# Jonetz/TreeDetection

Hardware: AMD Instinct MI355X
Metric: tiles/sec (1000x1000 RGB+nDSM) predict_tiles model stage (higher is better)
Workload: dtype f32

## Files before the change

### include/treedet.h

```cpp
#ifndef TREEDET_H
#define TREEDET_H

#include <stddef.h>
#include <stdint.h>

#ifdef __cplusplus
extern "C" {
#endif

typedef int td_status;
typedef struct td_engine td_engine;

enum {
    TD_OK = 0,
    TD_ERR_INVALID = -1,
    TD_ERR_HIP = -2,
    TD_ERR_WEIGHTS = -3,
    TD_ERR_CAPACITY = -4,
    TD_ERR_STATE = -5,
    TD_ERR_UNSUPPORTED = -6
};

enum { TD_PRECISION_FP32 = 0, TD_PRECISION_FP16 = 1 };
enum { TD_INPUT_F32_CHW = 0,
// ... 40 lines not shown
                            const int32_t* hw_out, int B, int Hp, int Wp, void* stream, td_detections* out);
#define TD_PHASE_STEM 6
td_status td_engine_forward_phase(td_engine* e, int phase, const void* images, int input_format, const int32_t* hw_valid,
                                  const int32_t* hw_out, int B, int Hp, int Wp, void* stream, td_detections* out);
td_status td_engine_tensor(td_engine* e, const char* name, void** dev_ptr, int64_t dims[4], int* elem_size);
td_status td_engine_read_tensor(td_engine* e, const char* name, void* dst_dev, int64_t bytes, void* stream);
#define TD_PROF_CATEGORIES 9
td_status td_engine_profile_enable(td_engine* e, int enable);
td_status td_engine_profile_read(td_engine* e, double* ms, int64_t* launches, double* flops, double* bytes, int reset);
#define TD_PROF_CLASSES 7
#define TD_CLS_WINO_GEMM 0
#define TD_CLS_WINO_XFORM 1
#define TD_CLS_CONV1X1 2
#define TD_CLS_CONV3X3 3
#define TD_CLS_FC 4
#define TD_CLS_MASK_HEAD 5
#define TD_CLS_TAIL 6
#define TD_PEAK_F32_MFMA_TFLOPS 157.3
#define TD_PEAK_F16_MFMA_TFLOPS 2500.0
#define TD_HBM_ACHIEVABLE_TBS 6.3
td_status td_engine_profile_classes(td_engine* e, double* ms, int64_t* launches, double* exec_flops, double* bytes, double* tmin_ms, int reset);
const char* td_last_error(void);
void td_engine_destroy(td_engine* e);

td_status td_resize_tile_u8(const uint8_t* src, int h, int w, int c, uint8_t* dst, int out_h, int out_w,
                            int dst_pitch_px, void* tmp_dev , void* stream);
td_status td_resize_batch_u8(const uint8_t* const* src_tiles, int n, int h, int w, int c, uint8_t* dst, int out_h,
                             int out_w, int dst_pitch_px, int64_t dst_image_stride_bytes, void* tmp_dev, void* stream);
td_status td_resize_bilinear_f64(const double* src, int c, int h, int w, float* dst, int out_h, int out_w, int dst_pitch_px,
                                 int64_t dst_plane_stride, void* stream);
td_status td_windows_u16_to_input(const uint16_t* raster, int height, int width, int c, const int32_t* windows, int n, int32_t* band1_max,
                                  float* dst, int out_h, int out_w, int dst_pitch_px, int64_t dst_plane_stride, int64_t dst_image_stride,
                                  void* stream);
void td_resize_shape(int h, int w, int short_edge, int max_size, int* out_h, int* out_w);

td_status td_bottleneck_tail_nhwc(const void* x, const void* w2, const float* scale2, const float* bias2, const void* w3,
                                  const float* scale3, const float* bias3, const void* shortcut, void* y, int B, int H, int W,
                                  int mid, int cout, int precision, void* stream);
td_status td_conv2d_nhwc(const void* x, const void* w, const float* scale, const float* bias,
                         const void* residual, int res_shift, void* y, int B, int H, int W, int Cin,
                         int Cout, int KH, int KW, int stride, int pad, int relu, int precision,
                         void* stream);
td_status td_conv2d_head_nhwc(const void* x, const void* w, const float* bias, const void* head_w, const float* head_b,
                              float* head_y, int B, int H, int W, int Cin, int KH, int KW, int pad, int head_n, int precision,
                              void* stream);
td_status td_conv2d_winograd_nhwc(const float* x, const float* w, const float* scale, const float* bias, float* y, int B,
                                  int H, int W, int Cin, int Cout, int relu, void* stream);
td_status td_conv2d_winograd_head_nhwc(const float* x, const float* w, const float* bias, const float* head_w, const float* head_b,
                                       float* head_y, int B, int H, int W, int Cin, int head_n, void* stream);
td_status td_nms(const float* boxes, const float* scores, int n, float iou_thresh, int32_t* keep_idx,
                 int32_t* keep_count, void* stream);
td_status td_roi_align(const void* feat, int H, int W, int C, const float* rois, int R, float spatial_scale,
                       int pooled, void* out, int precision, void* stream);
td_status td_paste_masks(const float* mask_probs, const float* boxes, int n, int out_h, int out_w,
                         float thresh, int32_t* mask_region, int64_t* mask_offset, uint32_t* mask_bits,
                         int64_t mask_words_cap, void* stream);

td_status td_paste_masks_batch(const float* mask_probs, const float* boxes, const int32_t* counts, const int32_t* out_hw,
                               int batch, int dets_per_image, float thresh, int32_t* mask_region, int64_t* mask_offset,
                               uint32_t* mask_bits, int64_t mask_words_per_image, void* stream);

#define TD_CONTOUR_MAX 256
td_status td_trace_contours_dev(const int32_t* mask_region, const int64_t* mask_offset, const uint32_t* mask_bits,
                                int64_t mask_words_per_image, const int32_t* counts, int batch, int dets_per_image,
                                int16_t* points, int points_cap, int32_t* image_points, int32_t* det_info,
                                int32_t* contour_info, void* stream);

int td_find_contours(const uint8_t* img, int h, int w, int32_t* points, int max_points, int32_t* starts,
                     int max_contours);
int td_tile_polygons_json(const int32_t* mask_region, const int64_t* mask_offset, const uint32_t* mask_bits,
                          int64_t mask_words, const float* scores, const int32_t* classes, int n,
                          const double* transform, const char* image_id, char* buf, int64_t cap, int64_t* needed);

int td_tile_prediction_file(int device, const int32_t* mask_region, const int64_t* mask_offset, const uint32_t* mask_bits_dev,
                            uint32_t* rows_host, int64_t mask_words, const float* scores, const int32_t* classes, int n,
                            const double* transform, const char* image_id, const char* path, int64_t* bytes_written);

int td_batch_prediction_files(int device, int n_tiles, int dets_per_image, const int32_t* mask_region, const int64_t* mask_offset,
                              const uint32_t* mask_bits_dev, uint32_t* rows_host, int64_t bits_stride_words, const float* scores,
                              const int32_t* classes, const int32_t* counts, const double* transforms, const char* image_id,
                              const char* const* paths, int threads, int32_t* status, int64_t* bytes_written);

int64_t td_tiff_lzw_decode(const uint8_t* src, int64_t n, uint8_t* dst, int64_t cap);
int64_t td_tiff_packbits_decode(const uint8_t* src, int64_t n, uint8_t* dst, int64_t cap);
int64_t td_tiff_lzw_encode(const uint8_t* src, int64_t n, uint8_t* dst, int64_t cap);
td_status td_tiff_lzw_decode_dev(const uint8_t* comp, const int64_t* block_off, const int64_t* block_nbytes, int nblocks,
                                 uint8_t* blocks_out, int64_t block_cap, int64_t* decoded, int32_t* status, void* stream);
td_status td_tiff_inflate_dev(const uint8_t* comp, const int64_t* block_off, const int64_t* block_nbytes, int nblocks,
                              uint8_t* blocks_out, int64_t block_cap, int64_t* decoded, int32_t* status, void* stream);
td_status td_tiff_inflate_verified_dev(const uint8_t* comp, const int64_t* block_off, const int64_t* block_nbytes, int nblocks,
                                       uint8_t* blocks_out, int64_t block_cap, int64_t* decoded, int32_t* status, int64_t* end_off,
                                       void* stream);
td_status td_tiff_adler32_blocks_dev(const uint8_t* blocks, int64_t block_cap, const int64_t* decoded, const uint8_t* comp,
                                     const int64_t* block_off, const int64_t* block_nbytes, const int64_t* end_off, int nblocks,
                                     int32_t* status, void* stream);
td_status td_adler32_dev(const uint8_t* data_dev, int64_t n, uint32_t* out_dev, void* stream);
int64_t td_tiff_inflate(const uint8_t* src, int64_t n, uint8_t* dst, int64_t cap);
int64_t td_tiff_inflate_verified(const uint8_t* src, int64_t n, uint8_t* dst, int64_t cap);
td_status td_tiff_blocks_to_image_dev(const uint8_t* blocks, int64_t block_cap, int block_w, int block_h, int blocks_across,
                                      int blocks_down, int spp, int predictor, uint8_t* image, int width, int height, void* stream);
td_status td_tiff_blocks_to_image_u16_dev(const uint8_t* blocks, int64_t block_cap, int block_w, int block_h, int blocks_across,
                                          int blocks_down, int spp, int predictor, uint16_t* image, int width, int height, void* stream);
td_status td_tiff_blocks_to_image_f32_dev(const uint8_t* blocks, int64_t block_cap, int block_w, int block_h, int blocks_across,
                                          int blocks_down, int spp, int predictor, float* image, int width, int height, void* stream);
#define TD_JPEG_TABSET_BYTES 11904
td_status td_tiff_jpeg_plan(const uint8_t* tables, int64_t tables_len, const uint8_t* data, const int64_t* block_off,
// ... 55 lines not shown
```

### treedetection_amd/_lib.py

```python
from __future__ import annotations

import ctypes as C
import os
import threading
from typing import Optional

_HERE = os.path.dirname(os.path.abspath(__file__))
LIB_PATH = os.path.join(_HERE, "libtreedet_hip.so")

_lib: Optional[C.CDLL] = None
ERR_INVALID = -1
ERR_CAPACITY = -4
ERR_STATE = -5
ERR_UNSUPPORTED = -6
JPEG_TABSET_BYTES = 11904
SAMPLE_U8, SAMPLE_F32 = 0, 1
RESAMPLE_MODES = {"f32": 0, "u8": 1, "ndvi": 2}


class TdError(RuntimeError):
    """A libtreedet_hip call returned a negative status (message from td_last_error)."""


class ModelDesc(C.Structure):
    _fields_ = [("num_classes", C.c_int32), ("precision", C.c_int32), ("pre_nms_topk", C.c_int32),
                ("post_nms_topk", C.c_int32), ("detections_per_image", C.c_int32),
                ("rpn_nms_thresh", C.c_float), ("score_thresh", C.c_float), ("nms_thresh", C.c_float),
                ("mask_thresh", C.c_float)]


class TensorDesc(C.Structure):
    _fields_ = [("name", C.c_char_p), ("data", C.c_void_p), ("ndim", C.c_int32), ("shape", C.c_int64 * 4)]


class Detections(C.Structure):
    _fields_ = [("boxes", C.c_void_p), ("scores", C.c_void_p), ("classes", C.c_void_p), ("count", C.c_void_p),
                ("mask_probs", C.c_void_p), ("mask_region", C.c_void_p), ("mask_offset", C.c_void_p),
                ("mask_bits", C.c_void_p), ("mask_words_per_image", C.c_int64)]


SIGNATURES = {
    "td_model_desc_default": (None, [C.POINTER(ModelDesc)]),
    "td_engine_create": (C.c_int, [C.POINTER(ModelDesc), C.c_int, C.POINTER(C.c_void_p)]),
    "td_engine_load_weights": (C.c_int, [C.c_void_p, C.POINTER(TensorDesc), C.c_size_t]),
    "td_engine_reserve": (C.c_int, [C.c_void_p, C.c_int, C.c_int, C.c_int]),
    "td_engine_forward": (C.c_int, [C.c_void_p, C.c_void_p, C.c_int, C.POINTER(C.c_int32), C.POINTER(C.c_int32),
                                    C.c_int, C.c_int, C.c_int, C.c_void_p, C.POINTER(Detections)]),
    "td_engine_forward_phase": (C.c_int, [C.c_void_p, C.c_int, C.c_void_p, C.c_int, C.POINTER(C.c_int32), C.POINTER(C.c_int32),
                                          C.c_int, C.c_int, C.c_int, C.c_void_p, C.POINTER(Detections)]),
    "td_engine_tensor": (C.c_int, [C.c_void_p, C.c_char_p, C.POINTER(C.c_void_p), C.POINTER(C.c_int64),
                                   C.POINTER(C.c_int)]),
    "td_engine_read_tensor": (C.c_int, [C.c_void_p, C.c_char_p, C.c_void_p, C.c_int64, C.c_void_p]),
    "td_engine_profile_enable": (C.c_int, [C.c_void_p, C.c_int]),
    "td_engine_profile_read": (C.c_int, [C.c_void_p, C.POINTER(C.c_double), C.POINTER(C.c_int64), C.POINTER(C.c_double),
                                         C.POINTER(C.c_double), C.c_int]),
    "td_engine_profile_classes": (C.c_int, [C.c_void_p, C.POINTER(C.c_double), C.POINTER(C.c_int64), C.POINTER(C.c_double),
                                            C.POINTER(C.c_double), C.POINTER(C.c_double), C.c_int]),
    "td_last_error": (C.c_char_p, []),
    "td_engine_destroy": (None, [C.c_void_p]),
    "td_resize_tile_u8": (C.c_int, [C.c_void_p, C.c_int, C.c_int, C.c_int, C.c_void_p, C.c_int, C.c_int, C.c_int,
                                    C.c_void_p, C.c_void_p]),
    "td_resize_batch_u8": (C.c_int, [C.POINTER(C.c_void_p), C.c_int, C.c_int, C.c_int, C.c_int, C.c_void_p, C.c_int, C.c_int,
                                     C.c_int, C.c_int64, C.c_void_p, C.c_void_p]),
    "td_bottleneck_tail_nhwc": (C.c_int, [C.c_void_p] * 9 + [C.c_int] * 6 + [C.c_void_p]),
    "td_resize_bilinear_f64": (C.c_int, [C.c_void_p, C.c_int, C.c_int, C.c_int, C.c_void_p, C.c_int, C.c_int, C.c_int, C.c_int64, C.c_void_p]),
    "td_windows_u16_to_input": (C.c_int, [C.c_void_p, C.c_int, C.c_int, C.c_int, C.c_void_p, C.c_int, C.c_void_p, C.c_void_p, C.c_int, C.c_int,
                                          C.c_int, C.c_int64, C.c_int64, C.c_void_p]),
    "td_resize_shape": (None, [C.c_int, C.c_int, C.c_int, C.c_int, C.POINTER(C.c_int), C.POINTER(C.c_int)]),
    "td_conv2d_nhwc": (C.c_int, [C.c_void_p, C.c_void_p, C.c_void_p, C.c_void_p, C.c_void_p, C.c_int, C.c_void_p]
                       + [C.c_int] * 11 + [C.c_void_p]),
    "td_conv2d_head_nhwc": (C.c_int, [C.c_void_p] * 6 + [C.c_int] * 9 + [C.c_void_p]),
    "td_conv2d_winograd_head_nhwc": (C.c_int, [C.c_void_p] * 6 + [C.c_int] * 5 + [C.c_void_p]),
    "td_conv2d_winograd_nhwc": (C.c_int, [C.c_void_p] * 5 + [C.c_int] * 6 + [C.c_void_p]),
    "td_nms": (C.c_int, [C.c_void_p, C.c_void_p, C.c_int, C.c_float, C.c_void_p, C.c_void_p, C.c_void_p]),
    "td_roi_align": (C.c_int, [C.c_void_p, C.c_int, C.c_int, C.c_int, C.c_void_p, C.c_int, C.c_float, C.c_int,
                               C.c_void_p, C.c_int, C.c_void_p]),
    "td_paste_masks": (C.c_int, [C.c_void_p, C.c_void_p, C.c_int, C.c_int, C.c_int, C.c_float, C.c_void_p,
                                 C.c_void_p, C.c_void_p, C.c_int64, C.c_void_p]),
    "td_paste_masks_batch": (C.c_int, [C.c_void_p, C.c_void_p, C.c_void_p, C.POINTER(C.c_int32), C.c_int, C.c_int, C.c_float,
                                       C.c_void_p, C.c_void_p, C.c_void_p, C.c_int64, C.c_void_p]),
    "td_crown_stats": (C.c_int, [C.c_void_p, C.c_int, C.c_int, C.POINTER(C.c_double), C.POINTER(C.c_int32), C.c_void_p, C.c_int,
                                 C.c_int, C.c_float, C.c_void_p, C.c_void_p]),
    "td_resample_gdal_dev": (C.c_int, [C.c_void_p, C.c_int, C.c_int, C.c_int, C.c_int, C.POINTER(C.c_int32), C.c_int]
                             + [C.c_void_p] * 4 + [C.c_int, C.c_int64] + [C.c_void_p] * 4 + [C.c_int, C.c_int64]
                             + [C.c_void_p, C.c_void_p, C.c_int, C.c_void_p]),
    "td_crown_pairs_count": (C.c_int, [C.c_void_p, C.c_void_p, C.c_int, C.c_float, C.c_uint16, C.c_void_p, C.c_float, C.c_void_p, C.c_void_p,
                                       C.c_void_p]),
    "td_crown_pairs_fill": (C.c_int, [C.c_void_p, C.c_void_p, C.c_int, C.c_float, C.c_uint16, C.c_void_p, C.c_void_p, C.c_void_p, C.c_void_p]),
    "td_crown_pairs_greedy": (C.c_int, [C.c_void_p, C.c_void_p, C.c_void_p, C.c_void_p, C.c_int, C.c_void_p]),
    "td_trace_contours_dev": (C.c_int, [C.c_void_p, C.c_void_p, C.c_void_p, C.c_int64, C.c_void_p, C.c_int, C.c_int, C.c_void_p,
                                        C.c_int, C.c_void_p, C.c_void_p, C.c_void_p, C.c_void_p]),
    "td_find_contours": (C.c_int, [C.c_void_p, C.c_int, C.c_int, C.c_void_p, C.c_int, C.c_void_p, C.c_int]),
    "td_batch_prediction_files": (C.c_int, [C.c_int, C.c_int, C.c_int, C.c_void_p, C.c_void_p, C.c_void_p, C.c_void_p, C.c_int64, C.c_void_p,
                                          C.c_void_p, C.c_void_p, C.c_void_p, C.c_char_p, C.POINTER(C.c_char_p), C.c_int, C.c_void_p, C.c_void_p]),
    "td_tiff_lzw_decode": (C.c_int64, [C.c_void_p, C.c_int64, C.c_void_p, C.c_int64]),
    "td_tiff_packbits_decode": (C.c_int64, [C.c_void_p, C.c_int64, C.c_void_p, C.c_int64]),
    "td_tiff_lzw_encode": (C.c_int64, [C.c_void_p, C.c_int64, C.c_void_p, C.c_int64]),
    "td_tiff_inflate": (C.c_int64, [C.c_void_p, C.c_int64, C.c_void_p, C.c_int64]),
    "td_tiff_inflate_dev": (C.c_int, [C.c_void_p, C.c_void_p, C.c_void_p, C.c_int, C.c_void_p, C.c_int64, C.c_void_p, C.c_void_p, C.c_void_p]),
    "td_tiff_inflate_verified": (C.c_int64, [C.c_void_p, C.c_int64, C.c_void_p, C.c_int64]),
    "td_tiff_inflate_verified_dev": (C.c_int, [C.c_void_p, C.c_void_p, C.c_void_p, C.c_int, C.c_void_p, C.c_int64, C.c_void_p, C.c_void_p, C.c_void_p,
                                               C.c_void_p]),
    "td_tiff_adler32_blocks_dev": (C.c_int, [C.c_void_p, C.c_int64, C.c_void_p, C.c_void_p, C.c_void_p, C.c_void_p, C.c_void_p, C.c_int, C.c_void_p,
                                             C.c_void_p]),
    "td_adler32_dev": (C.c_int, [C.c_void_p, C.c_int64, C.c_void_p, C.c_void_p]),
    "td_tiff_lzw_decode_dev": (C.c_int, [C.c_void_p, C.c_void_p, C.c_void_p, C.c_int, C.c_void_p, C.c_int64, C.c_void_p, C.c_void_p, C.c_void_p]),
    "td_tiff_blocks_to_image_dev": (C.c_int, [C.c_void_p, C.c_int64, C.c_int, C.c_int, C.c_int, C.c_int, C.c_int, C.c_int, C.c_void_p, C.c_int, C.c_int, C.c_void_p]),
    "td_tiff_blocks_to_image_u16_dev": (C.c_int, [C.c_void_p, C.c_int64, C.c_int, C.c_int, C.c_int, C.c_int, C.c_int, C.c_int, C.c_void_p, C.c_int,
                                                  C.c_int, C.c_void_p]),
    "td_tiff_blocks_to_image_f32_dev": (C.c_int, [C.c_void_p, C.c_int64, C.c_int, C.c_int, C.c_int, C.c_int, C.c_int, C.c_int, C.c_void_p, C.c_int,
                                                  C.c_int, C.c_void_p]),
    "td_tiff_jpeg_plan": (C.c_int, [C.c_void_p, C.c_int64, C.c_void_p, C.c_void_p, C.c_void_p, C.c_int, C.c_int, C.c_int, C.c_int, C.c_void_p,
                                    C.c_void_p, C.c_void_p, C.c_int64, C.c_void_p, C.c_int64, C.c_void_p]),
    "td_tiff_jpeg_decode_dev": (C.c_int, [C.c_void_p, C.c_void_p, C.c_int, C.c_void_p, C.c_int, C.c_void_p, C.c_void_p, C.c_void_p, C.c_int64,
                                          C.c_void_p, C.c_void_p] + [C.c_int] * 6 + [C.c_void_p]),
    "td_jpeg_decode": (C.c_int64, [C.c_void_p, C.c_int64, C.c_void_p, C.c_int64, C.c_void_p]),
    "td_read_windows": (C.c_int64, [C.c_int, C.c_int, C.c_void_p, C.c_int64, C.c_void_p, C.c_void_p, C.c_void_p, C.c_void_p, C.c_int]),
    "td_tiff_unpredict": (C.c_int, [C.c_void_p, C.c_int64, C.c_int64, C.c_int, C.c_int]),
    "td_tiff_unpredict_float": (C.c_int, [C.c_void_p, C.c_int64, C.c_int64, C.c_int, C.c_int]),
    "td_region_relate": (C.c_int, [C.c_void_p, C.c_void_p, C.c_void_p, C.c_int, C.c_void_p, C.c_void_p, C.c_int, C.c_void_p]),
    "td_simplify_ring": (C.c_int, [C.c_void_p, C.c_int, C.c_double, C.c_void_p, C.c_int]),
    "td_ring_is_valid": (C.c_int, [C.c_void_p, C.c_int]),
    "td_stitch_tile_json": (C.c_int, [C.c_char_p, C.c_int64, C.POINTER(C.c_double), C.c_double, C.c_int32, C.c_void_p,
                                      C.c_int64, C.c_void_p, C.c_void_p, C.c_int, C.POINTER(C.c_int64), C.POINTER(C.c_int)]),
    "td_stitch_tile_files": (C.c_int, [C.c_char_p, C.c_void_p, C.c_int, C.c_void_p, C.c_double, C.c_void_p, C.c_int, C.c_void_p, C.c_int64,
                                       C.c_void_p, C.c_void_p, C.c_int, C.c_void_p, C.POINTER(C.c_int64), C.POINTER(C.c_int)]),
    "td_tile_polygons_json_dev": (C.c_int, [C.c_void_p, C.c_int64, C.c_void_p, C.c_void_p, C.c_void_p, C.c_void_p, C.c_void_p, C.c_int64,
                                            C.c_void_p, C.c_void_p, C.c_int, C.POINTER(C.c_double), C.c_char_p, C.c_void_p, C.c_int64,
                                            C.POINTER(C.c_int64)]),
# ... 71 lines not shown
```

### treedetection_amd/csrc/api.cpp

```cpp
#include "common.h"
#include "detect.h"
#include <cstdarg>
#include <cstdio>
#include <cmath>
#include <cstdlib>
#include <vector>


namespace {
td_status scratch(void** p, size_t bytes) {
    TD_HIP_CHECK(hipMalloc(p, bytes ? bytes : 16));
    return TD_OK;
}
}

extern "C" {

void td_model_desc_default(td_model_desc* d) {
    d->num_classes = 1;
    d->precision = TD_PRECISION_FP32;
    d->pre_nms_topk = 1000;
    d->post_nms_topk = 1000;
    d->detections_per_image = 100;
    d->rpn_nms_thresh = 0.7f;
// ... 179 lines not shown
    const double scale = (double)short_edge / (double)(h < w ? h : w);
    double newh, neww;
    if (h < w) { newh = short_edge; neww = scale * w; }
    else { newh = scale * h; neww = short_edge; }
    const double mx = newh > neww ? newh : neww;
    if (mx > max_size) {
        const double s2 = (double)max_size / mx;
        newh *= s2;
        neww *= s2;
    }
    *out_h = (int)(newh + 0.5);
    *out_w = (int)(neww + 0.5);
}

td_status td_nms(const float* boxes, const float* scores, int n, float iou_thresh, int32_t* keep_idx,
                 int32_t* keep_count, void* stream) {
    TD_REQUIRE(boxes && scores && keep_idx && keep_count, "td_nms: null pointer");
    TD_REQUIRE(n >= 0 && n <= 32768, "td_nms: n=%d must be in [0, 32768]", n);
    hipStream_t s = static_cast<hipStream_t>(stream);
    if (n == 0) {
        TD_HIP_CHECK(hipMemsetAsync(keep_count, 0, sizeof(int32_t), s));
        return TD_OK;
    }
    void *sb = nullptr, *ss = nullptr, *si = nullptr, *sc = nullptr, *mk = nullptr, *kp = nullptr;
    td_status st;
    if ((st = scratch(&sb, sizeof(float) * 4 * n)) < 0) return st;
    if ((st = scratch(&ss, sizeof(float) * n)) < 0) return st;
    if ((st = scratch(&si, sizeof(int) * n)) < 0) return st;
    if ((st = scratch(&sc, sizeof(int))) < 0) return st;
    if ((st = scratch(&mk, sizeof(unsigned long long) * n * td_cdiv(n, 64))) < 0) return st;
    if ((st = scratch(&kp, sizeof(int) * n)) < 0) return st;
    if (n > 1024) {
        st = nms_big_launch(boxes, scores, n, iou_thresh, (float*)sb, (float*)ss, (int*)si, (int*)sc, (unsigned long long*)mk, (int*)kp, keep_count, s);
    } else {
        st = sort_boxes_launch(boxes, scores, nullptr, nullptr, 1, n, (float*)sb, (float*)ss, (int*)si, (int*)sc, s);
        if (st >= 0) st = nms_launch((float*)sb, (int*)sc, nullptr, 1, n, iou_thresh, (unsigned long long*)mk, (int*)kp, keep_count, n, s);
    }
    if (st >= 0) st = gather_keep_launch((int*)si, (int*)kp, keep_count, n, keep_idx, s);
    hipError_t herr = hipStreamSynchronize(s);
    (void)hipFree(sb); (void)hipFree(ss); (void)hipFree(si); (void)hipFree(sc); (void)hipFree(mk); (void)hipFree(kp);
    if (st < 0) return st;
    TD_HIP_CHECK(herr);
    return TD_OK;
}

td_status td_roi_align(const void* feat, int H, int W, int C, const float* rois, int R, float spatial_scale,
                       int pooled, void* out, int precision, void* stream) {
    TD_REQUIRE(feat && rois && out, "td_roi_align: null pointer");
    TD_REQUIRE(H >= 1 && W >= 1 && pooled >= 1 && R >= 0, "td_roi_align: bad geometry");
    if (R == 0) return TD_OK;
    return roi_align_single_launch(feat, H, W, C, rois, R, spatial_scale, pooled, out, precision, static_cast<hipStream_t>(stream));
}

td_status td_paste_masks(const float* mask_probs, const float* boxes, int n, int out_h, int out_w, float thresh,
                         int32_t* mask_region, int64_t* mask_offset, uint32_t* mask_bits, int64_t mask_words_cap,
                         void* stream) {
    TD_REQUIRE(mask_probs && boxes && mask_region && mask_offset && mask_bits, "td_paste_masks: null pointer");
    TD_REQUIRE(n >= 0 && n <= 1024 && out_h >= 1 && out_w >= 1, "td_paste_masks: bad shape");
    if (n == 0) return TD_OK;
    hipStream_t s = static_cast<hipStream_t>(stream);
    void* cnt = nullptr;
    td_status st = scratch(&cnt, sizeof(int));
    if (st < 0) return st;
    TD_HIP_CHECK(hipMemcpy(cnt, &n, sizeof(int), hipMemcpyHostToDevice));
    ImgSizes outsz{};
    outsz.h[0] = out_h;
    outsz.w[0] = out_w;
    st = paste_masks_launch(mask_probs, boxes, (int*)cnt, outsz, 1, n, thresh, mask_region,
                            reinterpret_cast<long long*>(mask_offset), mask_bits, mask_words_cap, s);
    hipError_t herr = hipStreamSynchronize(s);
    (void)hipFree(cnt);
    if (st < 0) return st;
    TD_HIP_CHECK(herr);
    return TD_OK;
}

td_status td_paste_masks_batch(const float* mask_probs, const float* boxes, const int32_t* counts, const int32_t* out_hw,
                               int batch, int dets_per_image, float thresh, int32_t* mask_region, int64_t* mask_offset,
                               uint32_t* mask_bits, int64_t mask_words_per_image, void* stream) {
    TD_REQUIRE(mask_probs && boxes && counts && out_hw && mask_region && mask_offset && mask_bits,
               "td_paste_masks_batch: null pointer");
    TD_REQUIRE(batch >= 1 && batch <= TD_MAX_BATCH && dets_per_image >= 1 && dets_per_image <= 1024,
               "td_paste_masks_batch: batch %d (max %d) / detections per image %d (max 1024)", batch, TD_MAX_BATCH, dets_per_image);
    ImgSizes outsz{};
    for (int i = 0; i < batch; ++i) {
        TD_REQUIRE(out_hw[2 * i] >= 1 && out_hw[2 * i + 1] >= 1, "td_paste_masks_batch: bad output size of image %d", i);
        outsz.h[i] = out_hw[2 * i];
        outsz.w[i] = out_hw[2 * i + 1];
        const int64_t need = (int64_t)dets_per_image * ((outsz.w[i] + 2 + 31) / 32) * outsz.h[i];
        TD_REQUIRE(mask_words_per_image >= need, "td_paste_masks_batch: image %d needs %lld mask words, capacity %lld", i,
                   (long long)need, (long long)mask_words_per_image);
    }
    return paste_masks_launch(mask_probs, boxes, counts, outsz, batch, dets_per_image, thresh, mask_region,
                              reinterpret_cast<long long*>(mask_offset), mask_bits, mask_words_per_image,
                              static_cast<hipStream_t>(stream));
}

}
```

### treedetection_amd/csrc/roi.hip

```cpp
#include "common.h"
#include "detect.h"
#include <cstdlib>
#include <type_traits>

namespace {

typedef _Float16 h4 __attribute__((ext_vector_type(4)));
__device__ __forceinline__ float4 load4(const float* p) { return *reinterpret_cast<const float4*>(p); }
__device__ __forceinline__ float4 load4(const _Float16* p) {
    const h4 v = *reinterpret_cast<const h4*>(p);
    return make_float4((float)v[0], (float)v[1], (float)v[2], (float)v[3]);
}
__device__ __forceinline__ void store4(float* p, const float4& v) { *reinterpret_cast<float4*>(p) = v; }
__device__ __forceinline__ void store4(_Float16* p, const float4& v) {
    h4 h;
    h[0] = (_Float16)v.x; h[1] = (_Float16)v.y; h[2] = (_Float16)v.z; h[3] = (_Float16)v.w;
    *reinterpret_cast<h4*>(p) = h;
}

__device__ __forceinline__ int fpn_level(float x1, float y1, float x2, float y2) {
    const float area = __fmul_rn(__fsub_rn(x2, x1), __fsub_rn(y2, y1));
    const float s = sqrtf(area);
    float lv = floorf(__fadd_rn(4.f, log2f(__fadd_rn(__fdiv_rn(s, 224.f), 1e-8f))));
    lv = fminf(fmaxf(lv, 2.f), 5.f);
// ... 13 lines not shown
    int gh, gw, ghw;
    float sh, sw, bh, bw;
    float count;
    size_t feat_off;
    int lvl;
};

__device__ __forceinline__ bool roi_setup(const FeatLevels& fl, const float* __restrict__ rois, const int* __restrict__ counts,
                                          int items, int roi_stride, int pooled, int compact, int* __restrict__ total_rows,
                                          int single_level, int item, int r, RoiGeo& g) {
    const int cnt = counts ? counts[item] : roi_stride;
    int prefix = 0;
    if (compact) {
        for (int i = 0; i < item; ++i) prefix += counts[i];
        if (blockIdx.x == 0 && blockIdx.y == 0 && threadIdx.x == 0 && total_rows) {
            int t = 0;
            for (int i = 0; i < items; ++i) t += counts[i];
            *total_rows = t;
        }
    }
    if (r >= cnt) return false;
    g.row = compact ? (size_t)(prefix + r) : (size_t)item * roi_stride + r;
    const float4 bx = *reinterpret_cast<const float4*>(rois + ((size_t)item * roi_stride + r) * 4);
    g.lvl = single_level ? 0 : fpn_level(bx.x, bx.y, bx.z, bx.w);
    g.H = fl.h[g.lvl];
    g.W = fl.w[g.lvl];
    const float sc = fl.scale[g.lvl];
    g.feat_off = single_level ? 0 : (size_t)item * g.H * g.W * fl.C;
    g.sw = __fsub_rn(__fmul_rn(bx.x, sc), 0.5f);
    g.sh = __fsub_rn(__fmul_rn(bx.y, sc), 0.5f);
    const float ew = __fsub_rn(__fmul_rn(bx.z, sc), 0.5f), eh = __fsub_rn(__fmul_rn(bx.w, sc), 0.5f);
    const float rw = __fsub_rn(ew, g.sw), rh = __fsub_rn(eh, g.sh);
    g.bh = __fdiv_rn(rh, (float)pooled);
    g.bw = __fdiv_rn(rw, (float)pooled);
    int gh = (int)ceilf(__fdiv_rn(rh, (float)pooled)), gw = (int)ceilf(__fdiv_rn(rw, (float)pooled));
    g.gh = gh > 0 ? gh : 0;
    g.gw = gw > 0 ? gw : 0;
    g.ghw = g.gh * g.gw;
    g.count = (float)(g.ghw > 1 ? g.ghw : 1);
    return true;
}

__device__ __forceinline__ bool roi_sample(float start, float bin, int p, int i, int g, int size, int& lo, int& hi, float& l, float& h) {
    const float c = __fadd_rn(__fadd_rn(start, __fmul_rn((float)p, bin)), __fdiv_rn(__fmul_rn(__fadd_rn((float)i, 0.5f), bin), (float)g));
    if (c < -1.f || c > (float)size) return false;
    float cc = c <= 0.f ? 0.f : c;
    lo = (int)cc;
    if (lo >= size - 1) { hi = lo = size - 1; cc = (float)lo; } else hi = lo + 1;
    l = __fsub_rn(cc, (float)lo);
    h = __fsub_rn(1.f, l);
    return true;
}

template <typename T, int D>
__global__ __launch_bounds__(256) void roi_align_kernel(FeatLevels fl, const float* __restrict__ rois,
                                                        const int* __restrict__ counts, int items, int roi_stride,
                                                        int pooled, int compact, T* __restrict__ out,
                                                        int* __restrict__ total_rows, int single_level, int parts) {
    const int item = blockIdx.y, r = blockIdx.x / parts, part = blockIdx.x - r * parts;
    RoiGeo geo;
    if (!roi_setup(fl, rois, counts, items, roi_stride, pooled, compact, total_rows, single_level, item, r, geo)) return;
    const size_t row = geo.row;
    const int H = geo.H, W = geo.W, C = fl.C, gh = geo.gh, gw = geo.gw, ghw = geo.ghw;
    const float sh = geo.sh, sw = geo.sw, bh = geo.bh, bw = geo.bw, count = geo.count;
    const T* __restrict__ feat = static_cast<const T*>(fl.feat[geo.lvl]) + geo.feat_off;

    constexpr int TAB = 14 * 24;
    __shared__ int t_lo[2][TAB], t_hi[2][TAB];
    __shared__ float t_l[2][TAB], t_h[2][TAB];
    const bool tab = pooled * gh <= TAB && pooled * gw <= TAB;
    if (tab) {
        for (int t = threadIdx.x; t < pooled * gh + pooled * gw; t += blockDim.x) {
            const int ax = t < pooled * gh ? 0 : 1;
            const int u = ax ? t - pooled * gh : t;
            const int g = ax ? gw : gh;
            const int p = u / g, i = u - p * g;
            int lo = 0, hi = 0;
            float l = 0.f, h = 0.f;
            const bool ok = ax ? roi_sample(sw, bw, p, i, g, W, lo, hi, l, h) : roi_sample(sh, bh, p, i, g, H, lo, hi, l, h);
            t_lo[ax][u] = ok ? lo : -1;
            t_hi[ax][u] = hi;
            t_l[ax][u] = l;
            t_h[ax][u] = h;
        }
        __syncthreads();
    }

    const int lane = threadIdx.x & 63, wave = __builtin_amdgcn_readfirstlane(threadIdx.x >> 6);
    const int nbins = pooled * pooled;
    const int g0 = part * 4 + wave, gstride = 4 * parts;
#define TD_RA(f) acc.f = __fadd_rn(acc.f, __fadd_rn(__fadd_rn(__fadd_rn(__fmul_rn(w1, v1.f), __fmul_rn(w2, v2.f)), __fmul_rn(w3, v3.f)), __fmul_rn(w4, v4.f)))
    if (tab && ghw > 0) {
        typedef typename Raw4<T>::type R4;
        const int nb_w = g0 < nbins ? (nbins - 1 - g0) / gstride + 1 : 0;
        const int total = nb_w * ghw;
        for (int cb = 0; cb < C; cb += 256) {
            const int c0 = cb + lane * 4;
            const bool act = c0 < C;
            int i_bin = g0, i_iy = 0, i_ix = 0, i_ph = g0 / pooled, i_pw = g0 - (g0 / pooled) * pooled;
            int c_bin = g0, c_n = 0;
            R4 v[D][4];
            float wgt[D][4];
            int ok[D];
            float4 acc = make_float4(0.f, 0.f, 0.f, 0.f);
            const int c0l = act ? c0 : 0;
            const int nb_all = nbins;
            auto issue = [&](int d) {
                const int ph = i_bin < nb_all ? i_ph : 0, pw = i_bin < nb_all ? i_pw : 0;
                const int yi = ph * gh + i_iy, xi = pw * gw + i_ix;
                const int yl = __builtin_amdgcn_readfirstlane(t_lo[0][yi]), xl = __builtin_amdgcn_readfirstlane(t_lo[1][xi]);
                const int yh = __builtin_amdgcn_readfirstlane(t_hi[0][yi]), xh = __builtin_amdgcn_readfirstlane(t_hi[1][xi]);
                ok[d] = yl >= 0 && xl >= 0;
                const float ly = t_l[0][yi], hy = t_h[0][yi], lx = t_l[1][xi], hx = t_h[1][xi];
                wgt[d][0] = __fmul_rn(hy, hx);
                wgt[d][1] = __fmul_rn(hy, lx);
                wgt[d][2] = __fmul_rn(ly, hx);
                wgt[d][3] = __fmul_rn(ly, lx);
                const int syl = ok[d] ? yl : 0, syh = ok[d] ? yh : 0, sxl = ok[d] ? xl : 0, sxh = ok[d] ? xh : 0;
                v[d][0] = *reinterpret_cast<const R4*>(feat + ((size_t)syl * W + sxl) * C + c0l);
                v[d][1] = *reinterpret_cast<const R4*>(feat + ((size_t)syl * W + sxh) * C + c0l);
                v[d][2] = *reinterpret_cast<const R4*>(feat + ((size_t)syh * W + sxl) * C + c0l);
                v[d][3] = *reinterpret_cast<const R4*>(feat + ((size_t)syh * W + sxh) * C + c0l);
                if (++i_ix == gw) {
                    i_ix = 0;
                    if (++i_iy == gh) {
                        i_iy = 0;
                        i_bin += gstride;
                        i_ph = i_bin / pooled;
                        i_pw = i_bin - i_ph * pooled;
                    }
                }
            };
            auto consume = [&](int d) {
                if (ok[d]) {
                    const float w1 = wgt[d][0], w2 = wgt[d][1], w3 = wgt[d][2], w4 = wgt[d][3];
                    const float4 v1 = widen4(v[d][0]), v2 = widen4(v[d][1]), v3 = widen4(v[d][2]), v4 = widen4(v[d][3]);
                    TD_RA(x); TD_RA(y); TD_RA(z); TD_RA(w);
                }
                if (++c_n == ghw) {
                    if (act) {
                        acc.x = __fdiv_rn(acc.x, count);
                        acc.y = __fdiv_rn(acc.y, count);
                        acc.z = __fdiv_rn(acc.z, count);
// ... 346 lines not shown
    const int x0 = rg[0], y0 = rg[1], x1 = rg[2], y1 = rg[3];
    const int wpr = (x1 - x0 + 31) >> 5, rows = y1 - y0;
    if (wpr <= 0 || rows <= 0) return;
    const float4 bx = *reinterpret_cast<const float4*>(boxes + ((size_t)b * D + d) * 4);
    const float bw = __fsub_rn(bx.z, bx.x), bh = __fsub_rn(bx.w, bx.y);
    uint32_t* out = bits + (size_t)b * words_per_image + offset[(size_t)b * D + d];
    for (int wi = threadIdx.x; wi < wpr * rows; wi += blockDim.x) {
        const int ry = wi / wpr, wx = wi - ry * wpr;
        const float py = __fadd_rn((float)(y0 + ry), 0.5f);
        const float gy = __fsub_rn(__fmul_rn(__fdiv_rn(__fsub_rn(py, bx.y), bh), 2.f), 1.f);
        const float iy = __fdiv_rn(__fsub_rn(__fmul_rn(__fadd_rn(gy, 1.f), (float)MS), 1.f), 2.f);
        const float iy0f = floorf(iy);
        const float wn = __fsub_rn(__fadd_rn(iy0f, 1.f), iy), ws = __fsub_rn(iy, iy0f);
        const int iy0 = (int)iy0f, iy1 = iy0 + 1;
        const bool yok0 = iy0 >= 0 && iy0 < MS, yok1 = iy1 >= 0 && iy1 < MS;
        uint32_t word = 0u;
        for (int bit = 0; bit < 32; ++bit) {
            const int x = x0 + wx * 32 + bit;
            if (x >= x1) break;
            const float px = __fadd_rn((float)x, 0.5f);
            const float gx = __fsub_rn(__fmul_rn(__fdiv_rn(__fsub_rn(px, bx.x), bw), 2.f), 1.f);
            const float ix = __fdiv_rn(__fsub_rn(__fmul_rn(__fadd_rn(gx, 1.f), (float)MS), 1.f), 2.f);
            const float ix0f = floorf(ix);
            const float ww = __fsub_rn(__fadd_rn(ix0f, 1.f), ix), we = __fsub_rn(ix, ix0f);
            float v = 0.f;
            if (isfinite(ix) && isfinite(iy)) {
                const int ix0 = (int)ix0f, ix1 = ix0 + 1;
                const bool xok0 = ix0 >= 0 && ix0 < MS, xok1 = ix1 >= 0 && ix1 < MS;
                const float nw = (yok0 && xok0) ? m[iy0 * MS + ix0] : 0.f;
                const float ne = (yok0 && xok1) ? m[iy0 * MS + ix1] : 0.f;
                const float sw = (yok1 && xok0) ? m[iy1 * MS + ix0] : 0.f;
                const float se = (yok1 && xok1) ? m[iy1 * MS + ix1] : 0.f;
                v = __fmul_rn(nw, __fmul_rn(wn, ww));
                v = __fadd_rn(v, __fmul_rn(ne, __fmul_rn(wn, we)));
                v = __fadd_rn(v, __fmul_rn(sw, __fmul_rn(ws, ww)));
                v = __fadd_rn(v, __fmul_rn(se, __fmul_rn(ws, we)));
            }
            if (v >= thresh) word |= 1u << bit;
        }
        out[(size_t)ry * wpr + wx] = word;
    }
}

}

static bool roi_h8_ok(const FeatLevels& fl) {
    static const char* env = getenv("TD_ROI_H8");
    if (env && atoi(env) == 0) return false;
    for (int l = 0; l < ROI_LEVELS; ++l)
        if ((size_t)fl.h[l] * (size_t)fl.w[l] * (size_t)fl.C >= ((size_t)1 << 32)) return false;
    return fl.C <= 256 && fl.C % 8 == 0;
}

template <typename T>
static void roi_align_dispatch(dim3 grid, hipStream_t stream, int depth, const FeatLevels& fl, const float* rois, const int* counts,
                               int items, int roi_stride, int pooled, int compact, T* out, int* total_rows, int single_level, int parts) {
    if constexpr (std::is_same<T, _Float16>::value) {
        if (roi_h8_ok(fl)) {
#define TD_ROI_LAUNCH8(DD) hipLaunchKernelGGL((roi_align_h8_kernel<DD>), grid, dim3(256), 0, stream, fl, rois, counts, items, \
                                              roi_stride, pooled, compact, out, total_rows, single_level, parts)
            switch (depth) {
                case 1: TD_ROI_LAUNCH8(1); break;
                case 3: TD_ROI_LAUNCH8(3); break;
                case 4: TD_ROI_LAUNCH8(4); break;
                default: TD_ROI_LAUNCH8(2); break;
            }
#undef TD_ROI_LAUNCH8
            return;
        }
    }
#define TD_ROI_LAUNCH(DD) hipLaunchKernelGGL((roi_align_kernel<T, DD>), grid, dim3(256), 0, stream, fl, rois, counts, items, \
                                             roi_stride, pooled, compact, out, total_rows, single_level, parts)
    switch (depth) {
        case 1: TD_ROI_LAUNCH(1); break;
        case 2: TD_ROI_LAUNCH(2); break;
        case 3: TD_ROI_LAUNCH(3); break;
        case 6: TD_ROI_LAUNCH(6); break;
        case 8: TD_ROI_LAUNCH(8); break;
        default: TD_ROI_LAUNCH(4); break;
    }
#undef TD_ROI_LAUNCH
}

static int roi_depth(int precision) {
    static const char* env = getenv("TD_ROI_DEPTH");
    if (env) return atoi(env);
    return precision == TD_PRECISION_FP16 ? 2 : 4;
}

static int roi_parts(int pooled) {
    static const char* env = getenv("TD_ROI_PARTS");
    if (env) return atoi(env) > 0 ? atoi(env) : 1;
    return pooled * pooled >= 128 ? 4 : 1;
}

td_status roi_align_launch(const FeatLevels& fl, const float* rois, const int* counts, int items, int roi_stride,
                           int pooled, int compact, void* out, int* total_rows, int precision, hipStream_t stream) {
    TD_REQUIRE(fl.C % 4 == 0, "roi_align: C must be a multiple of 4");
    const int parts = roi_parts(pooled);
    const dim3 grid(roi_stride * parts, items);
    if (precision == TD_PRECISION_FP16)
        roi_align_dispatch<_Float16>(grid, stream, roi_depth(precision), fl, rois, counts, items, roi_stride, pooled, compact,
                                     static_cast<_Float16*>(out), total_rows, 0, parts);
    else
        roi_align_dispatch<float>(grid, stream, roi_depth(precision), fl, rois, counts, items, roi_stride, pooled, compact,
                                  static_cast<float*>(out), total_rows, 0, parts);
    TD_KERNEL_CHECK();
    return TD_OK;
}

td_status roi_align_single_launch(const void* feat, int H, int W, int C, const float* rois, int R, float scale,
                                  int pooled, void* out, int precision, hipStream_t stream) {
    TD_REQUIRE(C % 4 == 0 && R >= 1, "roi_align: bad shape");
    FeatLevels fl{};
    fl.feat[0] = feat; fl.h[0] = H; fl.w[0] = W; fl.scale[0] = scale; fl.C = C;
    const int parts = roi_parts(pooled);
    const dim3 grid(R * parts, 1);
    if (precision == TD_PRECISION_FP16)
        roi_align_dispatch<_Float16>(grid, stream, roi_depth(precision), fl, rois, nullptr, 1, R, pooled, 0,
                                     static_cast<_Float16*>(out), nullptr, 1, parts);
    else
        roi_align_dispatch<float>(grid, stream, roi_depth(precision), fl, rois, nullptr, 1, R, pooled, 0,
                                  static_cast<float*>(out), nullptr, 1, parts);
    TD_KERNEL_CHECK();
    return TD_OK;
}

td_status det_decode_launch(const float* cls_reg, int cr_stride, const float* props, const int* prop_count,
                            const ImgSizes& valid, int B, int prop_stride, float score_thresh, float* boxes,
                            float* scores, int* flags, hipStream_t stream) {
    hipLaunchKernelGGL(det_decode_kernel, dim3(td_cdiv(B * prop_stride, 256)), dim3(256), 0, stream, cls_reg, cr_stride,
                       props, prop_count, valid, B, prop_stride, score_thresh, boxes, scores, flags);
    TD_KERNEL_CHECK();
    return TD_OK;
}

td_status det_finalize_launch(const float* sboxes, const float* sscores, const int* keep_pos, const int* keep_count,
                              const ImgSizes& valid, const ImgSizes& outsz, int B, int stride_items, int max_det,
                              float* det_boxes_net, float* out_boxes, float* out_scores, int* out_classes,
                              int* out_count, hipStream_t stream) {
    hipLaunchKernelGGL(det_finalize_kernel, dim3(B), dim3(64), 0, stream, sboxes, sscores, keep_pos, keep_count, valid,
                       outsz, stride_items, max_det, det_boxes_net, out_boxes, out_scores, out_classes, out_count);
    TD_KERNEL_CHECK();
    return TD_OK;
}

td_status mask_predict_launch(const void* x, const float* w, float bias, int C, int rows_max, const int* rows_dyn,
                              int rows_mul, float* logits_out, float* probs_out, int precision, hipStream_t stream) {
    TD_REQUIRE(C % 4 == 0, "mask_predict: C must be a multiple of 4");
    if (rows_max <= 0) return TD_OK;
    if (precision == TD_PRECISION_FP16)
        hipLaunchKernelGGL((mask_predict_kernel<_Float16>), dim3(td_cdiv(rows_max, 4)), dim3(256), 0, stream,
                           static_cast<const _Float16*>(x), w, bias, C, rows_max, rows_dyn, rows_mul, logits_out, probs_out);
    else
        hipLaunchKernelGGL((mask_predict_kernel<float>), dim3(td_cdiv(rows_max, 4)), dim3(256), 0, stream,
                           static_cast<const float*>(x), w, bias, C, rows_max, rows_dyn, rows_mul, logits_out, probs_out);
    TD_KERNEL_CHECK();
    return TD_OK;
}

td_status mask_scatter_launch(const float* compact, const int* counts, int B, int D, float* out, hipStream_t stream) {
    hipLaunchKernelGGL(mask_scatter_kernel, dim3(D, B), dim3(256), 0, stream, compact, counts, B, D, out);
    TD_KERNEL_CHECK();
    return TD_OK;
}

td_status paste_masks_launch(const float* probs, const float* boxes, const int* counts, const ImgSizes& outsz, int B,
                             int D, float thresh, int* region, long long* offset, uint32_t* bits,
                             long long words_per_image, hipStream_t stream) {
    hipLaunchKernelGGL(paste_plan_kernel, dim3(B), dim3(64), 0, stream, boxes, counts, outsz, D, region, offset,
                       words_per_image);
    TD_KERNEL_CHECK();
    hipLaunchKernelGGL(paste_fill_kernel, dim3(D, B), dim3(256), 0, stream, probs, boxes, counts, D, thresh, region,
                       offset, bits, words_per_image);
    TD_KERNEL_CHECK();
    return TD_OK;
// ... 2 lines not shown
```

Measured before the change: 678.8.

## Add streaming ROI-align path reusing column loads with LDS bin accumulators

Adds a streaming path to the FP32 ROI-align kernel for the case where the x sample table is monotone and densely covers a contiguous column range. Each feature column pair is loaded once per row and scattered into per-bin accumulators held in LDS, in runs of seven bins, instead of re-fetching four corners for every sample. The path is on by default and launches seven waves per block with dynamic LDS, replacing 256-thread blocks. It also exposes a multi-level ROI-align entry point in the C API and ctypes bindings. The trade-offs are more complex control flow, higher LDS use per block, and possibly different occupancy.

```diff
diff --git a/include/treedet.h b/include/treedet.h
--- a/include/treedet.h
+++ b/include/treedet.h
@@ -116,6 +116,9 @@
                  int32_t* keep_count, void* stream);
 td_status td_roi_align(const void* feat, int H, int W, int C, const float* rois, int R, float spatial_scale,
                        int pooled, void* out, int precision, void* stream);
+td_status td_roi_align_levels(const void* const feats[4], const int32_t h[4], const int32_t w[4], const float scale[4], int C,
+                              const float* rois, const int32_t* counts, int items, int roi_stride, int pooled, int compact,
+                              void* out, int32_t* total_rows, int precision, void* stream);
 td_status td_paste_masks(const float* mask_probs, const float* boxes, int n, int out_h, int out_w,
                          float thresh, int32_t* mask_region, int64_t* mask_offset, uint32_t* mask_bits,
                          int64_t mask_words_cap, void* stream);
diff --git a/treedetection_amd/_lib.py b/treedetection_amd/_lib.py
--- a/treedetection_amd/_lib.py
+++ b/treedetection_amd/_lib.py
@@ -75,6 +75,9 @@
     "td_nms": (C.c_int, [C.c_void_p, C.c_void_p, C.c_int, C.c_float, C.c_void_p, C.c_void_p, C.c_void_p]),
     "td_roi_align": (C.c_int, [C.c_void_p, C.c_int, C.c_int, C.c_int, C.c_void_p, C.c_int, C.c_float, C.c_int,
                                C.c_void_p, C.c_int, C.c_void_p]),
+    "td_roi_align_levels": (C.c_int, [C.POINTER(C.c_void_p), C.POINTER(C.c_int32), C.POINTER(C.c_int32), C.POINTER(C.c_float), C.c_int,
+                                      C.c_void_p, C.c_void_p, C.c_int, C.c_int, C.c_int, C.c_int, C.c_void_p, C.c_void_p, C.c_int,
+                                      C.c_void_p]),
     "td_paste_masks": (C.c_int, [C.c_void_p, C.c_void_p, C.c_int, C.c_int, C.c_int, C.c_float, C.c_void_p,
                                  C.c_void_p, C.c_void_p, C.c_int64, C.c_void_p]),
     "td_paste_masks_batch": (C.c_int, [C.c_void_p, C.c_void_p, C.c_void_p, C.POINTER(C.c_int32), C.c_int, C.c_int, C.c_float,
diff --git a/treedetection_amd/csrc/api.cpp b/treedetection_amd/csrc/api.cpp
--- a/treedetection_amd/csrc/api.cpp
+++ b/treedetection_amd/csrc/api.cpp
@@ -255,6 +255,22 @@
     return roi_align_single_launch(feat, H, W, C, rois, R, spatial_scale, pooled, out, precision, static_cast<hipStream_t>(stream));
 }
 
+td_status td_roi_align_levels(const void* const feats[4], const int32_t h[4], const int32_t w[4], const float scale[4], int C,
+                              const float* rois, const int32_t* counts, int items, int roi_stride, int pooled, int compact,
+                              void* out, int32_t* total_rows, int precision, void* stream) {
+    TD_REQUIRE(feats && h && w && scale && rois && out, "td_roi_align_levels: null pointer");
+    TD_REQUIRE(items >= 1 && roi_stride >= 1 && pooled >= 1 && C >= 4, "td_roi_align_levels: bad geometry");
+    TD_REQUIRE(!compact || counts, "td_roi_align_levels: compact rows need counts");
+    FeatLevels fl{};
+    for (int l = 0; l < ROI_LEVELS; ++l) {
+        TD_REQUIRE(feats[l] && h[l] >= 1 && w[l] >= 1, "td_roi_align_levels: bad level");
+        fl.feat[l] = feats[l]; fl.h[l] = h[l]; fl.w[l] = w[l]; fl.scale[l] = scale[l];
+    }
+    fl.C = C;
+    return roi_align_launch(fl, rois, counts, items, roi_stride, pooled, compact, out, total_rows, precision,
+                            static_cast<hipStream_t>(stream));
+}
+
 td_status td_paste_masks(const float* mask_probs, const float* boxes, int n, int out_h, int out_w, float thresh,
                          int32_t* mask_region, int64_t* mask_offset, uint32_t* mask_bits, int64_t mask_words_cap,
                          void* stream) {
diff --git a/treedetection_amd/csrc/roi.hip b/treedetection_amd/csrc/roi.hip
--- a/treedetection_amd/csrc/roi.hip
+++ b/treedetection_amd/csrc/roi.hip
@@ -89,11 +89,15 @@
     return true;
 }
 
+constexpr int ROI_RUN = 7;
+extern __shared__ float4 roi_acc_lds[];
+
 template <typename T, int D>
-__global__ __launch_bounds__(256) void roi_align_kernel(FeatLevels fl, const float* __restrict__ rois,
+__global__ __launch_bounds__(512) void roi_align_kernel(FeatLevels fl, const float* __restrict__ rois,
                                                         const int* __restrict__ counts, int items, int roi_stride,
                                                         int pooled, int compact, T* __restrict__ out,
-                                                        int* __restrict__ total_rows, int single_level, int parts) {
+                                                        int* __restrict__ total_rows, int single_level, int parts,
+                                                        int stream_on) {
     const int item = blockIdx.y, r = blockIdx.x / parts, part = blockIdx.x - r * parts;
     RoiGeo geo;
     if (!roi_setup(fl, rois, counts, items, roi_stride, pooled, compact, total_rows, single_level, item, r, geo)) return;
@@ -125,7 +129,168 @@
 
     const int lane = threadIdx.x & 63, wave = __builtin_amdgcn_readfirstlane(threadIdx.x >> 6);
     const int nbins = pooled * pooled;
-    const int g0 = part * 4 + wave, gstride = 4 * parts;
+    const int nw = blockDim.x >> 6;
+    const int g0 = part * nw + wave, gstride = nw * parts;
+
+    int k0 = 0, k1 = 0;
+    bool stream = false;
+    if (stream_on && tab && ghw > 0) {
+        const int nx = pooled * gw;
+        int first = nx, last = -1, nok = 0;
+        bool mono = true;
+        for (int base = 0; base < nx; base += 64) {
+            const int idx = base + lane;
+            const int lo = idx < nx ? t_lo[1][idx] : -1;
+            const int nxt = idx + 1 < nx ? t_lo[1][idx + 1] : -1;
+            const unsigned long long okm = __ballot(lo >= 0);
+            const unsigned long long bad = __ballot(lo >= 0 && nxt >= 0 && nxt < lo);
+            if (okm) {
+                if (first == nx) first = base + __ffsll(okm) - 1;
+                last = base + 63 - __clzll(okm);
+                nok += __popcll(okm);
+            }
+            mono = mono && bad == 0ull;
+        }
+        if (nok > 0 && mono && last - first + 1 == nok) {
+            k0 = first;
+            k1 = last + 1;
+            const int xmin = __builtin_amdgcn_readfirstlane(t_lo[1][first]), xmax = __builtin_amdgcn_readfirstlane(t_hi[1][last]);
+            stream = xmax - xmin + 1 <= 2 * nok;
+        }
+    }
+    if (stream) {
+        typedef typename Raw4<T>::type R4;
+        constexpr int DC = 2 * D;
+        const int nruns = (pooled + ROI_RUN - 1) / ROI_RUN, units = pooled * nruns;
+        float4* __restrict__ sacc = roi_acc_lds + wave * (ROI_RUN * 64) + lane;
+#define TD_RS(f) s.f = __fadd_rn(__fadd_rn(__fadd_rn(__fmul_rn(w1, v1.f), __fmul_rn(w2, v2.f)), __fmul_rn(w3, v3.f)), __fmul_rn(w4, v4.f))
+        for (int cb = 0; cb < C; cb += 256) {
+            const int c0 = cb + lane * 4;
+            const bool act = c0 < C;
+            const int c0l = act ? c0 : 0;
+            for (int u = g0; u < units; u += gstride) {
+                const int ph = u / nruns, b0 = (u - ph * nruns) * ROI_RUN;
+                const int nb = pooled - b0 < ROI_RUN ? pooled - b0 : ROI_RUN;
+                const int ka = k0 > b0 * gw ? k0 : b0 * gw, kb = k1 < (b0 + nb) * gw ? k1 : (b0 + nb) * gw;
+                const bool any = ka < kb;
+                const int kf = any ? ka : k0;
+                const int xa = __builtin_amdgcn_readfirstlane(t_lo[1][kf]);
+                const int xb = any ? __builtin_amdgcn_readfirstlane(t_hi[1][kb - 1]) : xa;
+                const int ncols = xb - xa + 1;
+                const int total = any ? gh * ncols : 0;
+                const int pa = kf / gw - b0, ixa = kf - (kf / gw) * gw;
+#pragma unroll
+                for (int p = 0; p < ROI_RUN; ++p) sacc[p * 64] = make_float4(0.f, 0.f, 0.f, 0.f);
+                float4 acc = make_float4(0.f, 0.f, 0.f, 0.f);
+                int acc_p = -1;
+                R4 vt[DC], vb[DC];
+                vt[DC - 1] = R4{};
+                vb[DC - 1] = R4{};
+                int i_iy = 0, i_col = 0;
+                const T* i_top = feat;
+                const T* i_bot = feat;
+                auto i_rows = [&]() {
+                    const int yi = ph * gh + (i_iy < gh ? i_iy : 0);
+                    const int yl = __builtin_amdgcn_readfirstlane(t_lo[0][yi]), yh = __builtin_amdgcn_readfirstlane(t_hi[0][yi]);
+                    const int syl = yl >= 0 ? yl : 0, syh = yl >= 0 ? yh : 0;
+                    i_top = feat + ((size_t)syl * W + xa) * C + c0l;
+                    i_bot = feat + ((size_t)syh * W + xa) * C + c0l;
+                };
+                auto issue = [&](int d) {
+                    vt[d] = *reinterpret_cast<const R4*>(i_top + (size_t)i_col * C);
+                    vb[d] = *reinterpret_cast<const R4*>(i_bot + (size_t)i_col * C);
+                    if (++i_col == ncols) {
+                        i_col = 0;
+                        ++i_iy;
+                        i_rows();
+                    }
+                };
+                int c_iy = 0, c_col = xa;
+                int k = kf, kp = pa, kix = ixa;
+                int e_lo = 0, e_hi = 0;
+                float e_l = 0.f, e_h = 0.f, ly = 0.f, hy = 0.f;
+                bool yok = false;
+                auto c_rows = [&]() {
+                    const int yi = ph * gh + (c_iy < gh ? c_iy : 0);
+                    yok = __builtin_amdgcn_readfirstlane(t_lo[0][yi]) >= 0;
+                    ly = t_l[0][yi];
+                    hy = t_h[0][yi];
+                };
+                auto fetch = [&]() {
+                    const int kk = k < kb ? k : kf;
+                    e_lo = __builtin_amdgcn_readfirstlane(t_lo[1][kk]);
+                    e_hi = k < kb ? __builtin_amdgcn_readfirstlane(t_hi[1][kk]) : 0x7fffffff;
+                    e_l = t_l[1][kk];
+                    e_h = t_h[1][kk];
+                };
+                auto consume = [&](int d) {
+                    const int pd = (d + DC - 1) % DC;
+                    if (yok) {
+                        while (e_hi == c_col) {
+                            const bool same = e_lo == e_hi;
+                            const float lx = e_l, hx = e_h;
+                            if (kp != acc_p) {
+                                if (acc_p >= 0) sacc[acc_p * 64] = acc;
+                                acc = sacc[kp * 64];
+                                acc_p = kp;
+                            }
+                            ++k;
+                            if (++kix == gw) {
+                                kix = 0;
+                                ++kp;
+                            }
+                            fetch();
+                            const float w1 = __fmul_rn(hy, hx), w2 = __fmul_rn(hy, lx), w3 = __fmul_rn(ly, hx), w4 = __fmul_rn(ly, lx);
+                            const float4 v2 = widen4(vt[d]), v4 = widen4(vb[d]);
+                            const float4 v1 = same ? v2 : widen4(vt[pd]), v3 = same ? v4 : widen4(vb[pd]);
+                            float4 s;
+                            TD_RS(x); TD_RS(y); TD_RS(z); TD_RS(w);
+                            acc.x = __fadd_rn(acc.x, s.x);
+                            acc.y = __fadd_rn(acc.y, s.y);
+                            acc.z = __fadd_rn(acc.z, s.z);
+                            acc.w = __fadd_rn(acc.w, s.w);
+                        }
+                    }
+                    if (c_col == xb) {
+                        c_col = xa;
+                        k = kf; kp = pa; kix = ixa;
+                        fetch();
+                        ++c_iy;
+                        c_rows();
+                    } else {
+                        ++c_col;
+                    }
+                };
+                i_rows();
+                c_rows();
+                fetch();
+#pragma unroll
+                for (int d = 0; d < DC - 1; ++d) issue(d);
+                for (int t0 = 0; t0 < total; t0 += DC) {
+#pragma unroll
+                    for (int d = 0; d < DC; ++d) {
+                        if (t0 + d < total) consume(d);
+                        issue((d + DC - 1) % DC);
+                    }
+                }
+                if (acc_p >= 0) sacc[acc_p * 64] = acc;
+#pragma unroll
+                for (int p = 0; p < ROI_RUN; ++p) {
+                    if (p < nb && act) {
+                        float4 a = sacc[p * 64];
+                        a.x = __fdiv_rn(a.x, count);
+                        a.y = __fdiv_rn(a.y, count);
+                        a.z = __fdiv_rn(a.z, count);
+                        a.w = __fdiv_rn(a.w, count);
+                        store4(out + (row * nbins + (size_t)ph * pooled + b0 + p) * C + c0, a);
+                    }
+                }
+            }
+        }
+#undef TD_RS
+        return;
+    }
+
 #define TD_RA(f) acc.f = __fadd_rn(acc.f, __fadd_rn(__fadd_rn(__fadd_rn(__fmul_rn(w1, v1.f), __fmul_rn(w2, v2.f)), __fmul_rn(w3, v3.f)), __fmul_rn(w4, v4.f)))
     if (tab && ghw > 0) {
         typedef typename Raw4<T>::type R4;
@@ -578,11 +743,33 @@
     return fl.C <= 256 && fl.C % 8 == 0;
 }
 
+static int roi_depth(int precision) {
+    static const char* env = getenv("TD_ROI_DEPTH");
+    if (env) return atoi(env);
+    return precision == TD_PRECISION_FP16 ? 2 : 4;
+}
+
+static int roi_stream_waves() {
+    static const char* senv = getenv("TD_ROI_STREAM");
+    static const char* wenv = getenv("TD_ROI_WAVES");
+    if (senv && atoi(senv) == 0) return 0;
+    const int w = wenv ? atoi(wenv) : 7;
+    return w >= 1 && w <= 8 ? w : 7;
+}
+
+static int roi_parts(int pooled) {
+    static const char* env = getenv("TD_ROI_PARTS");
+    if (env) return atoi(env) > 0 ? atoi(env) : 1;
+    return pooled * pooled >= 128 ? 4 : 1;
+}
+
 template <typename T>
-static void roi_align_dispatch(dim3 grid, hipStream_t stream, int depth, const FeatLevels& fl, const float* rois, const int* counts,
-                               int items, int roi_stride, int pooled, int compact, T* out, int* total_rows, int single_level, int parts) {
+static void roi_align_dispatch(hipStream_t stream, int depth, const FeatLevels& fl, const float* rois, const int* counts,
+                               int items, int roi_stride, int pooled, int compact, T* out, int* total_rows, int single_level) {
     if constexpr (std::is_same<T, _Float16>::value) {
         if (roi_h8_ok(fl)) {
+            const int parts = roi_parts(pooled);
+            const dim3 grid(roi_stride * parts, items);
 #define TD_ROI_LAUNCH8(DD) hipLaunchKernelGGL((roi_align_h8_kernel<DD>), grid, dim3(256), 0, stream, fl, rois, counts, items, \
                                               roi_stride, pooled, compact, out, total_rows, single_level, parts)
             switch (depth) {
@@ -595,8 +782,12 @@
             return;
         }
     }
-#define TD_ROI_LAUNCH(DD) hipLaunchKernelGGL((roi_align_kernel<T, DD>), grid, dim3(256), 0, stream, fl, rois, counts, items, \
-                                             roi_stride, pooled, compact, out, total_rows, single_level, parts)
+    const int waves = roi_stream_waves(), stream_on = waves != 0;
+    const int parts = roi_parts(pooled);
+    const dim3 grid(roi_stride * parts, items), block(stream_on ? 64 * waves : 256);
+    const size_t lds = stream_on ? (size_t)waves * ROI_RUN * 64 * sizeof(float4) : 0;
+#define TD_ROI_LAUNCH(DD) hipLaunchKernelGGL((roi_align_kernel<T, DD>), grid, block, lds, stream, fl, rois, counts, items, roi_stride, pooled, \
+                                             compact, out, total_rows, single_level, parts, stream_on)
     switch (depth) {
         case 1: TD_ROI_LAUNCH(1); break;
         case 2: TD_ROI_LAUNCH(2); break;
@@ -608,29 +799,15 @@
 #undef TD_ROI_LAUNCH
 }
 
-static int roi_depth(int precision) {
-    static const char* env = getenv("TD_ROI_DEPTH");
-    if (env) return atoi(env);
-    return precision == TD_PRECISION_FP16 ? 2 : 4;
-}
-
-static int roi_parts(int pooled) {
-    static const char* env = getenv("TD_ROI_PARTS");
-    if (env) return atoi(env) > 0 ? atoi(env) : 1;
-    return pooled * pooled >= 128 ? 4 : 1;
-}
-
 td_status roi_align_launch(const FeatLevels& fl, const float* rois, const int* counts, int items, int roi_stride,
                            int pooled, int compact, void* out, int* total_rows, int precision, hipStream_t stream) {
     TD_REQUIRE(fl.C % 4 == 0, "roi_align: C must be a multiple of 4");
-    const int parts = roi_parts(pooled);
-    const dim3 grid(roi_stride * parts, items);
     if (precision == TD_PRECISION_FP16)
-        roi_align_dispatch<_Float16>(grid, stream, roi_depth(precision), fl, rois, counts, items, roi_stride, pooled, compact,
-                                     static_cast<_Float16*>(out), total_rows, 0, parts);
+        roi_align_dispatch<_Float16>(stream, roi_depth(precision), fl, rois, counts, items, roi_stride, pooled, compact,
+                                     static_cast<_Float16*>(out), total_rows, 0);
     else
-        roi_align_dispatch<float>(grid, stream, roi_depth(precision), fl, rois, counts, items, roi_stride, pooled, compact,
-                                  static_cast<float*>(out), total_rows, 0, parts);
+        roi_align_dispatch<float>(stream, roi_depth(precision), fl, rois, counts, items, roi_stride, pooled, compact,
+                                  static_cast<float*>(out), total_rows, 0);
     TD_KERNEL_CHECK();
     return TD_OK;
 }
@@ -640,14 +817,12 @@
     TD_REQUIRE(C % 4 == 0 && R >= 1, "roi_align: bad shape");
     FeatLevels fl{};
     fl.feat[0] = feat; fl.h[0] = H; fl.w[0] = W; fl.scale[0] = scale; fl.C = C;
-    const int parts = roi_parts(pooled);
-    const dim3 grid(R * parts, 1);
     if (precision == TD_PRECISION_FP16)
-        roi_align_dispatch<_Float16>(grid, stream, roi_depth(precision), fl, rois, nullptr, 1, R, pooled, 0,
-                                     static_cast<_Float16*>(out), nullptr, 1, parts);
+        roi_align_dispatch<_Float16>(stream, roi_depth(precision), fl, rois, nullptr, 1, R, pooled, 0,
+                                     static_cast<_Float16*>(out), nullptr, 1);
     else
-        roi_align_dispatch<float>(grid, stream, roi_depth(precision), fl, rois, nullptr, 1, R, pooled, 0,
-                                  static_cast<float*>(out), nullptr, 1, parts);
+        roi_align_dispatch<float>(stream, roi_depth(precision), fl, rois, nullptr, 1, R, pooled, 0,
+                                  static_cast<float*>(out), nullptr, 1);
     TD_KERNEL_CHECK();
     return TD_OK;
 }
```

New measurement: 675.3. No clear change (-0.5%).
